# diver-j/melgan-multi

Measured on NVIDIA H100. Metric: generator_fwd_audio_frames_per_sec, higher is better.
Workload: dtype f32 in/out; products as 3 split-bf16 wgmma passes with fp32 accumulation (fp32-equivalent, ~1e-5)

## Files before the change

include/melgan_b200.h:

```cpp
#ifndef MELGAN_B200_H_
#define MELGAN_B200_H_

#include <stddef.h>
#include <stdint.h>

#ifdef __cplusplus
extern "C" {
#endif

#define MG_OK 0
#define MG_ERR_INVALID_ARGUMENT (-1)
#define MG_ERR_CUDA (-2)
#define MG_ERR_UNSUPPORTED_DEVICE (-3)
#define MG_ERR_WORKSPACE_TOO_SMALL (-4)
#define MG_ERR_OUT_OF_MEMORY (-5)

#define MG_GEN_NUM_LAYERS 30

int mg_abi_version(void);

const char *mg_last_error_string(void);

int mg_device_check(void);

// ... 8 lines not shown
#define MG_GEN_RAGGED_MAX_B 256
int mg_gen_forward_ragged(const void *packed, const float *mel, float *audio, int B, int T_max, const int *lengths,
                          void *workspace, size_t workspace_bytes, void *stream);

int mg_gen_forward_timed(const void *packed, const float *mel, float *audio, int B, int T,
                         void *workspace, size_t workspace_bytes, void *stream, float *kernel_ms);

int mg_gen_check_status(const void *workspace, int B, int T, void *stream);

int mg_gen_convt(const void *packed, int stage, const float *x, float *y, int B, int Lin, void *stream);

int mg_gen_resblock(const void *packed, int stage, const float *x, float *y, int B, int L, void *stream);
int mg_gen_upres(const void *packed, int stage, const float *x, float *y, int B, int Lin, void *stream);
int mg_gen_upres_post(const void *packed, const float *x, float *audio, int B, int Lin, void *stream);
const char *mg_gen_resblock_config(int code);

int mg_gen_resup(const void *packed, int stage, const float *x, float *y, int B, int L, void *stream);

int mg_gen_conv_pre(const void *packed, const float *mel, float *y, int B, int T, void *stream);
int mg_gen_resblock_post(const void *packed, const float *x, float *audio, int B, int L, void *stream);

int mg_gen_resblock_trace(const void *packed, int stage, const float *x, float *y, int B, int L, long long *trace_host);

int mg_gen_stage_output(const void *workspace, int which, float *out, int B, int T, void *stream);

size_t mg_msd_packed_bytes(void);
int mg_msd_pack(const float *const *v, const float *const *g, const float *const *bias, void *packed, void *stream);
int mg_msd_lengths(int L, int *lens);
int mg_msd_forward(const void *packed, const float *y, int Bt, int L, float *const *fmaps, void *status_word, void *stream);
int mg_msd_check_status(const void *status_word, void *stream);
// ... 65 lines not shown
```

melgan_multi_b200/csrc/mg_api.cu:

```cuda
#include <new>
#include <stdlib.h>
#include <string.h>

#include "mg_common.cuh"

namespace mg {


static int *status_ptr(void *workspace, int B, int T) {
    return reinterpret_cast<int *>(reinterpret_cast<float *>(workspace) + ws_offset(6, (size_t)B, (size_t)T));
}

static int run_generator(const float *packed, const float *mel, float *audio, const RunTable &batch, float *ws, cudaStream_t s,
                         cudaEvent_t *ev, const float *mel_host = nullptr, float *audio_host = nullptr) {
    int *st = status_ptr(ws, batch.items(), batch.stride);
    MG_CUDA_TRY(cudaMemsetAsync(st, 0, sizeof(int), s));
    return launch_generator_tc(packed, mel, audio, batch, ws, st, s, ev, mel_host, audio_host);
}

static int check_shape(const char *fn, int B, int T) {
    if (B < 1 || T < 1) return set_error(MG_ERR_INVALID_ARGUMENT, "%s: need B >= 1 and T >= 1 (got B=%d, T=%d)", fn, B, T);
    if ((long long)B * T > (1ll << 24)) return set_error(MG_ERR_INVALID_ARGUMENT, "%s: B*T = %lld too large", fn, (long long)B * T);
    return MG_OK;
}
// ... 264 lines not shown
int mg_gen_conv_pre(const void *packed, const float *mel, float *y, int B, int T, void *stream) {
    if (!packed || !mel || !y || B < 1 || T < 1) return set_error(MG_ERR_INVALID_ARGUMENT, "mg_gen_conv_pre: bad argument");
    return run_one_kernel("mg_gen_conv_pre", (cudaStream_t)stream, [&](int *st) {
        return launch_gen_pre_tc(mel, y, (const float *)packed, RunTable::uniform(B, T), st, (cudaStream_t)stream);
    });
}

int mg_gen_resblock_post(const void *packed, const float *x, float *audio, int B, int L, void *stream) {
    if (!packed || !x || !audio || B < 1 || L < 1) return set_error(MG_ERR_INVALID_ARGUMENT, "mg_gen_resblock_post: bad argument");
    return run_one_kernel("mg_gen_resblock_post", (cudaStream_t)stream, [&](int *st) {
        return launch_resblock_tc(x, audio, (const float *)packed, 4, RunTable::uniform(B, L), st, (cudaStream_t)stream);
    });
}

int mg_gen_resblock_trace(const void *packed, int stage, const float *x, float *y, int B, int L, long long *trace_host) {
    if (!packed || !x || !y || x == y || !trace_host || stage < 0 || stage > 3)
        return set_error(MG_ERR_INVALID_ARGUMENT, "mg_gen_resblock_trace: bad argument");
    int *st = nullptr;
    long long *tr = nullptr;
    MG_CUDA_TRY(cudaMalloc(&st, sizeof(int)));
    MG_CUDA_TRY(cudaMalloc(&tr, 128 * sizeof(long long)));
    cudaMemset(st, 0, sizeof(int));
    cudaMemset(tr, 0, 128 * sizeof(long long));
    int rc = launch_resblock_tc(x, y, (const float *)packed, stage, RunTable::uniform(B, L), st, 0, tr);
    if (rc == MG_OK && cudaDeviceSynchronize() != cudaSuccess) rc = set_error(MG_ERR_CUDA, "mg_gen_resblock_trace: kernel failed");
    if (rc == MG_OK) cudaMemcpy(trace_host, tr, 128 * sizeof(long long), cudaMemcpyDeviceToHost);
    cudaFree(st);
    cudaFree(tr);
    return rc;
}

// ... 18 lines not shown
        return set_error(MG_ERR_INVALID_ARGUMENT, "mg_gen_upres: bad argument");
    return run_one_kernel("mg_gen_upres", (cudaStream_t)stream, [&](int *st) {
        return launch_resblock_tc(x, y, (const float *)packed, 10 + stage, RunTable::uniform(B, 2 * Lin), st, (cudaStream_t)stream);
    });
}

int mg_gen_upres_post(const void *packed, const float *x, float *audio, int B, int Lin, void *stream) {
    if (!packed || !x || !audio || (const void *)x == (const void *)audio || B < 1 || Lin < 1)
        return set_error(MG_ERR_INVALID_ARGUMENT, "mg_gen_upres_post: bad argument");
    return run_one_kernel("mg_gen_upres_post", (cudaStream_t)stream, [&](int *st) {
        return launch_resblock_tc(x, audio, (const float *)packed, 14, RunTable::uniform(B, 2 * Lin), st, (cudaStream_t)stream);
    });
}

const char *mg_gen_resblock_config(int code) { return resblock_config_name(code, 0); }


size_t mg_msd_packed_bytes(void) { return msd_packed_bytes(); }

int mg_msd_pack(const float *const *v, const float *const *g, const float *const *bias, void *packed, void *stream) {
    if (!v || !g || !bias || !packed) return set_error(MG_ERR_INVALID_ARGUMENT, "mg_msd_pack: null argument");
    if ((uintptr_t)packed % 256) return set_error(MG_ERR_INVALID_ARGUMENT, "mg_msd_pack: packed must be 256-byte aligned");
    return launch_disc_pack(v, g, bias, packed, (cudaStream_t)stream);
}

int mg_msd_lengths(int L, int *lens) {
    if (L < 1 || !lens) return set_error(MG_ERR_INVALID_ARGUMENT, "mg_msd_lengths: bad argument");
    msd_lengths(L, lens);
    for (int i = 0; i < 21; ++i)
        if (lens[i] < 1) return set_error(MG_ERR_INVALID_ARGUMENT, "mg_msd_lengths: L = %d is too short for the discriminators", L);
// ... 192 lines not shown
```

melgan_multi_b200/csrc/mg_common.cuh:

```cuda
#pragma once
#include <cuda_runtime.h>
#include <stdarg.h>
#include <stdint.h>
#include <stdio.h>

#include "../../include/melgan_b200.h"
#include "mg_layout.h"

namespace mg {

constexpr int kNumSMs = 132;

char *error_buffer();
int set_error(int code, const char *fmt, ...);

#define MG_CUDA_TRY(expr)                                                                     \
    do {                                                                                      \
        cudaError_t err__ = (expr);                                                           \
        if (err__ != cudaSuccess)                                                             \
            return ::mg::set_error(MG_ERR_CUDA, "%s failed: %s (%s:%d)", #expr,               \
                                   cudaGetErrorString(err__), __FILE__, __LINE__);            \
    } while (0)

__device__ __forceinline__ float lrelu(float x) { return fmaxf(x, x * kSlope); }
// ... 150 lines not shown
                            float *const *dg, cudaStream_t s);
int launch_adam(float *const *p, const float *const *g, float *const *m, float *const *v, const long long *n, const int *first,
                int count, int total_ctas, float lr, float b1, float b2, float eps, float wd, long long step, cudaStream_t s);
long long loss_num_ctas(const long long *n, int count);
int launch_loss_forward(const float *const *a, const float *const *b, const long long *n, const int *mode, int count, float *out,
                        float *partial, cudaStream_t s);
int launch_loss_backward(const float *const *a, const float *const *b, const long long *n, const int *mode, int count,
                         const float *gout, float *const *ga, float *const *gb, cudaStream_t s);
struct MelTables;
size_t mel_tables_bytes();
int mel_tables_build(int sr, int n_mels, float fmin, float fmax, int norm, MelTables *t);
int mel_frames(int L);
int launch_mel(const void *tables, const float *audio, float *mel, int B, int L, cudaStream_t s);
int launch_msd_forward(const void *packed, const float *y, int Bt, int L, float *const *fmaps, int *status, cudaStream_t s);
int launch_convt_tc(const float *x, float *y, const float *packed, int stage, const RunTable &batch, int *status, cudaStream_t s);
int launch_resblock_tc(const float *x, float *y, const float *packed, int stage, const RunTable &batch, int *status, cudaStream_t s,
                       long long *trace = nullptr);

}
```

melgan_multi_b200/csrc/mg_res_tc.cu:

```cuda
#include <stdlib.h>
#include <string.h>

#include "mg_common.cuh"
#include "mg_tc.cuh"

namespace mg {
using namespace tc;

template <int C_, int NRB_, int RPW_, int NCP_, int NSTAGE_, bool POST_ = false, bool UPF_ = false, int UPT_ = 0, int CS_ = 1>
struct RbCfg {
    static constexpr int C = C_, NRB = NRB_, RPW = RPW_, NCP = NCP_, NSTAGE = NSTAGE_, UPT = UPT_, CS = CS_;
    static constexpr bool POST = POST_;
    static constexpr bool UPF = UPF_;
    static constexpr int P = 64 * NRB;
    static constexpr int NWG = NRB / RPW * NCP;
    static constexpr int NCONS = 128 * NWG;
    static constexpr int NT = NCONS + 32;
    static constexpr int NCW = C / NCP;
    static constexpr int SLACK = 16;
    static constexpr int HALO = 16 + (POST ? 3 : 0);
    static constexpr int HL = HALO + (UPT_ ? 1 : 0);
    static constexpr int ROWS = P + 2 * SLACK;
    static constexpr int XPITCH = ROWS * 16;
    static constexpr int KP = C / 8;
// ... 3 lines not shown
    static constexpr int HALF = CHUNK / 2;
    static constexpr int NCHUNK = tc_chunks_per_conv(C);
    static constexpr int KSL = C / KC;
    static constexpr int TNG = UPT == 8 ? 32 : C / 2, TN = (UPT ? UPT : 1) * TNG, TNCG = (C / 2) / TNG;
    static constexpr int TSLOT = UPT == 8 ? 16384 : 128 * UPT * TNG, TNSLOT = UPT ? TNCG * (C / 16) * (UPT == 8 ? 2 : 1) : 0;
    static_assert(UPT == 0 || ((UPT == 2 || UPT == 8) && TN == C && TSLOT <= CHUNK && !POST_ && !UPF_), "tail ConvT shape");
    static_assert(UPT != 8 || NCW == 128, "stride-8 tail: each column part stores four phases of a channel as one float4");
    static constexpr int UROWS = P / 2 + 2, UPITCH = UROWS * 16, NPB = NRB / 2, UKSL = 2 * C / KC, NUPCH = UPF ? 4 * UKSL : 0;
    static constexpr int SPITCH = P + 4;
    static_assert(!UPF || (NCP == 1 && NPB <= NWG && 2 * KP * UPITCH <= XBYTES && C * SPITCH * 4 <= 2 * XBYTES),
                  "fused ConvT must fit the X region");
    static_assert(!POST || (C == 32 && NCP == 1), "conv_post fusion is for the 32-channel stage");
    static constexpr int PVB = CS * P - HALO - HL, XCH = 9;
    static_assert(CS == 1 || ((CS == 2 || CS == 4) && !POST_ && !UPF_ && UPT_ == 0 && XCH <= SLACK && 2 * XCH <= P),
                  "clusters are for the plain ResBlock");
    static constexpr int SMEM_BYTES = 2 * XBYTES + NSTAGE * CHUNK + 2 * C * 4 + (2 * NSTAGE + (CS > 1 ? 2 : 0) + 1) * 8;
    static_assert(SMEM_BYTES + 1024 <= 227 * 1024, "shared memory budget");
    static_assert(XPITCH / 16 < 16384, "LBO field");
    static_assert(NRB % RPW == 0 && C % NCP == 0 && NCW % 32 == 0, "warpgroup split");
};

template <int RPW, int R>
__device__ __forceinline__ void acc_fence2(float (&a)[RPW][R]) {
#pragma unroll
    for (int r = 0; r < RPW; ++r) acc_fence<R>(a[r]);
}

template <class Cfg>
__global__ void __launch_bounds__(Cfg::NT, 1)
resblock_tc_kernel(const float *__restrict__ x, float *__restrict__ y, const float *__restrict__ packed, int stage,
                   const __grid_constant__ RunTable clusters, int *__restrict__ status, long long *__restrict__ trace) {
    constexpr int C = Cfg::C, P = Cfg::P, SLACK = Cfg::SLACK, HALO = Cfg::HALO, HL = Cfg::HL;
    constexpr int XPITCH = Cfg::XPITCH, XBYTES = Cfg::XBYTES, KC = Cfg::KC, CHUNK = Cfg::CHUNK, NSTAGE = Cfg::NSTAGE;
    constexpr int NCONS = Cfg::NCONS, NCP = Cfg::NCP, NCW = Cfg::NCW, RPW = Cfg::RPW, KSL = Cfg::KSL, NA = NCW / 2;
    constexpr int CS = Cfg::CS, XCH = Cfg::XCH;
    extern __shared__ __align__(1024) uint8_t smem[];
    uint8_t *Xh = smem, *Xl = smem + XBYTES, *ring = smem + 2 * XBYTES;
    float *pend = reinterpret_cast<float *>(ring + NSTAGE * CHUNK);
    float *b1s = pend + C;
    uint64_t *full = reinterpret_cast<uint64_t *>(b1s + C);
    uint64_t *empty = full + NSTAGE;
    uint64_t *hfull = empty + NSTAGE, *hfree = hfull + 1;
    int *item_len = reinterpret_cast<int *>(empty + NSTAGE + (CS > 1 ? 2 : 0));

    const int tid = threadIdx.x, warp = tid >> 5, lane = tid & 31;
    const int crank = blockIdx.x % CS;
    const RunPos cp = clusters.find(blockIdx.x / CS);
    const int clus = cp.unit, Ls = clusters.stride;
    auto item = [&]() { return *reinterpret_cast<volatile int *>(&item_len[0]); };
    auto len = [&]() { return *reinterpret_cast<volatile int *>(&item_len[1]); };
    const int oc = clus == 0 ? 0 : (CS * P - HALO) + (clus - 1) * Cfg::PVB - HL;
    const int o = oc + crank * P;
    const int p_lo = (clus == 0 || crank > 0) ? 0 : HL, p_hi = (crank < CS - 1 || oc + CS * P >= cp.len) ? P : P - HALO;
    const bool interior = (o >= 0 && o + P <= cp.len);
    const int l0 = 5 + 6 * stage;
// ... 6 lines not shown
            mbar_init(&full[s], 1);
            mbar_init(&empty[s], Cfg::NWG * CS);
        }
        if constexpr (CS > 1) {
            mbar_init(hfull, 1);
            mbar_init(hfree, (crank > 0) + (crank < CS - 1));
        }
        fence_mbar_init();
    }
    for (int i = Cfg::UPF ? 1 << 30 : tid; i < 2 * Cfg::KP * 2 * SLACK; i += Cfg::NT) {
        const int r = i % (2 * SLACK), kp = (i / (2 * SLACK)) % Cfg::KP, hl = i / (2 * SLACK * Cfg::KP);
        const int row = r < SLACK ? r : P + r;
        *reinterpret_cast<uint4 *>((hl ? Xl : Xh) + kp * XPITCH + row * 16) = make_uint4(0, 0, 0, 0);
    }
    for (int i = tid; i < C; i += Cfg::NT) pend[i] = 0.f;
    fence_proxy_async();
    __syncthreads();
    if constexpr (CS > 1) cluster_sync();
    const bool tr = trace && blockIdx.x == (gridDim.x > 1 ? 1u : 0u) && tid == 0;
#define MG_TR(slot) do { if (tr) trace[slot] = clock64(); } while (0)

    if (warp == NCONS / 32) {
        if (lane == 0) {
            int s = 0, ph = 0, j = 0;
            bool ok = true;
            auto put = [&](const uint8_t *src, uint32_t bytes) {
                if (!ok || !mbar_wait(&empty[s], ph ^ 1)) { ok = false; return; }
                mbar_arrive_expect_tx(&full[s], bytes);
                if constexpr (CS == 1) bulk_g2s(ring + s * CHUNK, src, bytes, &full[s]);
                else if (j % CS == crank) bulk_g2s_multicast(ring + s * CHUNK, src, bytes, &full[s], (1 << CS) - 1);
// ... 186 lines not shown
                    for (int k16 = 0; k16 < KC / 16; ++k16) {
                        const uint64_t bdesc = bbase + (uint64_t)(((pass == 2 ? Cfg::HALF : 0) + 2 * k16 * (C * 16)) >> 4);
                        const uint64_t adesc = desc_at(udesc_t, (pass == 1 ? xl_addr : xh_addr) + arow + 2 * k16 * UPITCH);
                        wgmma_bf16<NCW>(A[0], adesc, bdesc, !(k < 2 && ks == 0 && pass == 0 && k16 == 0));
                    }
                chunk_end();
            }
        };
        upf_tap(D, 0);
        upf_tap(R, 1);
        upf_tap(D, 2);
        upf_tap(R, 3);
        drain();
        sync_cons();
        float *stg = reinterpret_cast<float *>(Xh);
        const float *ubias = packed + bias_offset(1 + stage);
        if (mine) {
#pragma unroll
            for (int h = 0; h < 2; ++h) {
                const int m = wgi * 64 + frag_row(t, h);
#pragma unroll
                for (int j = 0; j < NA; ++j) {
                    const int col = frag_col(q, (j & ~3) | (j & 1));
                    if ((j & 2) == 2 * h) {
                        const float bj = __ldg(ubias + col);
                        *reinterpret_cast<float2 *>(stg + (size_t)col * SPITCH + 2 * m) = make_float2(R[0][j] + bj, D[0][j] + bj);
                    }
                }
            }
        }
        sync_cons();
#pragma unroll
        for (int r = 0; r < RPW; ++r)
#pragma unroll
            for (int j = 0; j < NA; ++j) {
                const int p = (rb0 + r) * 64 + frag_row(t, (j >> 1) & 1);
                R[r][j] = stg[(size_t)frag_col(q, (j & ~3) | (j & 1)) * SPITCH + p];
            }
        sync_cons();
        for (int i = tid; i < 2 * Cfg::KP * 2 * SLACK; i += NCONS) {
// ... 10 lines not shown
                const int p = (rb0 + r) * 64 + frag_row(t, h), tp = o + p;
                const bool inr = (tp >= 0 && tp < L);
                const float *xp = x + (size_t)b * C * Ls + (inr ? tp : 0);
#pragma unroll
                for (int k = 0; k < NCW / 8; ++k)
#pragma unroll
                    for (int e = 0; e < 2; ++e)
                        R[r][4 * k + 2 * h + e] = inr ? __ldg(xp + (size_t)(c0 + frag_col(q, 4 * k + e)) * Ls) : 0.f;
            }
    }
    hand_off(R, pend, false);
    MG_TR(1);

#pragma unroll 1
    for (int pr = 0; pr < 3; ++pr) {
        const float *bias1 = packed + bias_offset(l0 + pr);
        for (int c = tid; c < C; c += NCONS) b1s[c] = __ldg(bias1 + c);
        MG_TR(2 + 6 * pr);
        conv_mma(D, pr == 0 ? 1 : pr == 1 ? 3 : 9, true, 2 * pr);
        MG_TR(3 + 6 * pr);
        x_read();
        hand_off(D, b1s, false);
        MG_TR(4 + 6 * pr);
        const float *bias2 = packed + bias_offset(l0 + 3 + pr);
        for (int c = tid; c < C; c += NCONS) pend[c] += __ldg(bias2 + c);
        MG_TR(5 + 6 * pr);
        conv_mma(R, 1, false, 2 * pr + 1);
        MG_TR(6 + 6 * pr);
        x_read();
        if (pr < 2 || Cfg::UPT != 0) hand_off(R, pend, Cfg::UPT != 0 && pr == 2);
        MG_TR(7 + 6 * pr);
    }

    if constexpr (Cfg::POST) {
        pdl_trigger();
        float *Q = reinterpret_cast<float *>(Xh);
        float *wpost = reinterpret_cast<float *>(Xl);
        for (int i = tid; i < 32 * 8; i += NCONS)
            wpost[i] = (i & 7) < kPostK ? __ldg(packed + weight_offset(29) + (i >> 3) * kPostK + (i & 7)) : 0.f;
        sync_cons();
#pragma unroll
        for (int r = 0; r < RPW; ++r)
#pragma unroll
            for (int h = 0; h < 2; ++h) {
                const int p = (rb0 + r) * 64 + frag_row(t, h), tp = o + p;
                const bool inr = (tp >= 0 && tp < len());
                float qk[kPostK];
#pragma unroll
                for (int k = 0; k < kPostK; ++k) qk[k] = 0.f;
#pragma unroll
                for (int k = 0; k < NCW / 8; ++k)
#pragma unroll
                    for (int e = 0; e < 2; ++e) {
                        const int ci = frag_col(q, 4 * k + e);
                        const float a = inr ? lrelu(R[r][4 * k + 2 * h + e] + pend[ci]) : 0.f;
// ... 3 lines not shown
                        qk[3] = fmaf(w0.w, a, qk[3]); qk[4] = fmaf(w1.x, a, qk[4]); qk[5] = fmaf(w1.y, a, qk[5]);
                        qk[6] = fmaf(w1.z, a, qk[6]);
                    }
#pragma unroll
                for (int k = 0; k < kPostK; ++k) {
                    qk[k] += __shfl_xor_sync(0xffffffffu, qk[k], 1);
                    qk[k] += __shfl_xor_sync(0xffffffffu, qk[k], 2);
                }
                if (q == 0) {
#pragma unroll
                    for (int k = 0; k < kPostK; ++k) Q[k * P + p] = qk[k];
                }
            }
        sync_cons();
        const int b = item(), L = len();
        const float bpost = __ldg(packed + bias_offset(29));
#pragma unroll 1
        for (int p = tid; p < P; p += NCONS) {
            const int tp = o + p;
            if (p >= p_lo && p < p_hi && tp < L) {
                float acc = bpost;
#pragma unroll
                for (int k = 0; k < kPostK; ++k) {
                    const int pp = p + k - 3;
                    if (pp >= 0 && pp < P) acc += Q[k * P + pp];
                }
                y[(size_t)b * Ls + tp] = tanhf(acc);
            }
        }
        if (oc + P >= L)
            for (int p = L + tid; p < Ls; p += NCONS) y[(size_t)b * Ls + p] = 0.f;
    } else if constexpr (Cfg::UPT != 0) {
        constexpr int S = Cfg::UPT, TNG = Cfg::TNG, TN = Cfg::TN, PADT = S / 2, COT = C / 2;
        const int b = item(), L = len();
        const int Lout = S * Ls;
        const float *tbias = packed + bias_offset(1 + stage + 1);
        {
            const int pl = L - 1 - o;
            if (pl >= p_lo && pl < p_hi) {
                const float *wf = packed + weight_offset(1 + stage + 1);
                for (int i = tid; i < PADT * COT; i += NCONS) {
                    const int co = i / PADT, j = i - co * PADT;
                    const float *wp = wf + ((size_t)co * S + j) * 2 + 1;
                    float acc0 = 0.f, acc1 = 0.f, acc2 = 0.f, acc3 = 0.f;
#pragma unroll 1
                    for (int cc = 0; cc < C; cc += 32) {
                        float wv[32];
#pragma unroll
                        for (int k = 0; k < 32; ++k) wv[k] = __ldg(wp + (size_t)(cc + k) * COT * S * 2);
#pragma unroll
                        for (int k = 0; k < 32; k += 4) {
                            acc0 = fmaf(b1s[cc + k], wv[k], acc0);
                            acc1 = fmaf(b1s[cc + k + 1], wv[k + 1], acc1);
                            acc2 = fmaf(b1s[cc + k + 2], wv[k + 2], acc2);
                            acc3 = fmaf(b1s[cc + k + 3], wv[k + 3], acc3);
                        }
                    }
                    y[((size_t)b * COT + co) * Lout + (size_t)S * L - PADT + j] = (acc0 + acc1) + (acc2 + acc3) + __ldg(tbias + co);
                }
            }
        }
        const uint64_t tbdesc_t = desc_template(TN * 16, 128);
#pragma unroll 1
        for (int cg = 0; cg < Cfg::TNCG; ++cg) {
#pragma unroll 1
            for (int ch = 0; ch < C / 16; ++ch) {
#pragma unroll 1
                for (int ts = 0; ts < (S == 8 ? 2 : 1); ++ts) {
                    const uint64_t bbase = desc_at(tbdesc_t, chunk_begin() + c0 * 16);
#pragma unroll
                    for (int tp = 0; tp < (S == 8 ? 1 : 2); ++tp) {
                        const int tap = S == 8 ? ts : tp;
#pragma unroll
// ... 15 lines not shown
#pragma unroll
            for (int r = 0; r < RPW; ++r)
#pragma unroll
                for (int h = 0; h < 2; ++h) {
                    const int p = (rb0 + r) * 64 + frag_row(t, h), sg = o + p;
                    const bool own = (p >= p_lo && p < p_hi && sg < L);
                    const bool lo_ok = own && sg >= 1, hi_ok = own;
                    if constexpr (S == 8) {
                        const bool ok8 = c0 == 0 ? lo_ok : hi_ok;
                        float *yb = y + ((size_t)b * COT + cg * TNG) * Lout + (own ? 8 * sg - PADT + (c0 >> 5) : 0);
#pragma unroll
                        for (int c = 0; c < 4; ++c)
#pragma unroll
                            for (int e = 0; e < 2; ++e) {
                                const int co = 8 * c + 2 * q + e;
                                const float bj = __ldg(tbias + cg * TNG + co);
                                if (ok8)
                                    *reinterpret_cast<float4 *>(yb + (size_t)co * Lout) =
                                        make_float4(D[r][4 * c + 2 * h + e] + bj, D[r][4 * (4 + c) + 2 * h + e] + bj,
                                                    D[r][4 * (8 + c) + 2 * h + e] + bj, D[r][4 * (12 + c) + 2 * h + e] + bj);
                            }
                    } else {
                        float *yb = y + (size_t)b * COT * Lout + (own ? 2 * sg - PADT : 0);
#pragma unroll
                        for (int k = 0; k < NCW / 8; ++k)
#pragma unroll
                            for (int e = 0; e < 2; ++e) {
                                const int col = c0 + frag_col(q, 4 * k + e), phi = col / TNG, co = col % TNG;
                                if (phi == 0 ? lo_ok : hi_ok) yb[(size_t)co * Lout + phi] = D[r][4 * k + 2 * h + e] + __ldg(tbias + co);
                            }
                    }
                }
        }
    } else {
        pdl_trigger();
        const int b = item(), L = len();
#pragma unroll
        for (int r = 0; r < RPW; ++r)
#pragma unroll
            for (int h = 0; h < 2; ++h) {
                const int p = (rb0 + r) * 64 + frag_row(t, h), tp = o + p;
                if (p >= p_lo && p < p_hi && tp < L) {
                    float *yp = y + (size_t)b * C * Ls + tp;
#pragma unroll
// ... 106 lines not shown
```

melgan_multi_b200/csrc/mg_up_tc.cu:

```cuda
#include "mg_common.cuh"
#include "mg_tc.cuh"

namespace mg {
using namespace tc;

template <int STAGE_>
struct UpCfg {
    static constexpr int STAGE = STAGE_;
    static constexpr int CIN = stage_cin(STAGE), COUT = stage_cout(STAGE), S = stage_stride(STAGE), PAD = stage_pad(STAGE);
    static constexpr int NG = up_ng(STAGE);
    static constexpr int NCG = COUT / NG;
    static constexpr int N = S * NG;
    static constexpr int NMW = (N > 128) ? 1 : 2;
    static constexpr int KCA = (S == 8) ? 64 : 32;
    static constexpr int ROWS = 64 * NMW;
    static constexpr int AROWS = ROWS + 8;
    static constexpr int APITCH = AROWS * 16;
    static constexpr int ASLOT = 2 * (KCA / 8) * APITCH;
    static constexpr int BSLOT = up_slot_bytes(STAGE);
    static constexpr int NSA = (CIN == KCA) ? 1 : 2, NSB = (S == 8) ? 4 : (CIN >= 128 ? 2 : 3);
    static constexpr int NCHUNK = CIN / 16;
    static constexpr int NCONV = 128;
    static constexpr int NT = NCONV + 128 * NMW + 32;
    static constexpr int SMEM_BYTES = NSA * ASLOT + NSB * BSLOT + (2 * NSA + 2 * NSB) * 8;
    static_assert(N <= 256 && N % 16 == 0, "wgmma N");
    static_assert(SMEM_BYTES + 1024 <= 227 * 1024, "shared memory budget");
    static_assert(CIN % KCA == 0, "A slot");
};

template <class Cfg, class Row>
__device__ __forceinline__ void convt_store(const float *acc, float *__restrict__ y, const float *__restrict__ bias, int mw, int t,
                                            int cg, int Lout, Row row) {
    constexpr int S = Cfg::S, NG = Cfg::NG, N = Cfg::N, COUT = Cfg::COUT, PAD = Cfg::PAD;
    const int q = t & 3;
#pragma unroll
    for (int h = 0; h < 2; ++h) {
        int m = 64 * mw + frag_row(t, h);
        asm volatile("" : "+r"(m) : : "memory");
        const RunPos p = row(m);
        const int s = p.unit;
        const bool row_ok = p.item >= 0;
        const bool lo_ok = row_ok && s >= 1, hi_ok = row_ok && s <= p.len - 1;
        float *yb = y + ((size_t)(row_ok ? p.item : 0) * COUT + cg * NG) * Lout + (S * s - PAD);
        if constexpr (S == 8) {
#pragma unroll
            for (int c = 0; c < 4; ++c)
#pragma unroll
                for (int e = 0; e < 2; ++e) {
                    const int co = 8 * c + 2 * q + e;
                    const float bj = __ldg(bias + co);
                    float *yp = yb + (size_t)co * Lout;
                    if (lo_ok)
                        *reinterpret_cast<float4 *>(yp) =
                            make_float4(acc[4 * (0 + c) + 2 * h + e] + bj, acc[4 * (4 + c) + 2 * h + e] + bj,
                                        acc[4 * (8 + c) + 2 * h + e] + bj, acc[4 * (12 + c) + 2 * h + e] + bj);
                    if (hi_ok)
                        *reinterpret_cast<float4 *>(yp + 4) =
                            make_float4(acc[4 * (16 + c) + 2 * h + e] + bj, acc[4 * (20 + c) + 2 * h + e] + bj,
                                        acc[4 * (24 + c) + 2 * h + e] + bj, acc[4 * (28 + c) + 2 * h + e] + bj);
                }
        } else {
#pragma unroll
            for (int k = 0; k < N / 8; ++k)
#pragma unroll
                for (int e = 0; e < 2; ++e) {
                    const int col = frag_col(q, 4 * k + e), phi = col / NG, co = col % NG;
                    const float o = acc[4 * k + 2 * h + e] + __ldg(bias + co);
                    if (phi == 0 ? lo_ok : hi_ok) yb[(size_t)co * Lout + phi] = o;
                }
        }
    }
}

template <class Cfg>
__global__ void __launch_bounds__(Cfg::NT, 1)
convt_tc_kernel(const float *__restrict__ x, float *__restrict__ y, const float *__restrict__ packed,
                const __grid_constant__ RunTable rows, int *__restrict__ status) {
    constexpr int CIN = Cfg::CIN, N = Cfg::N, NG = Cfg::NG;
    constexpr int ROWS = Cfg::ROWS, APITCH = Cfg::APITCH, ASLOT = Cfg::ASLOT, BSLOT = Cfg::BSLOT, KCA = Cfg::KCA;
    constexpr int NSA = Cfg::NSA, NSB = Cfg::NSB, NCHUNK = Cfg::NCHUNK, NCONV = Cfg::NCONV, NMW = Cfg::NMW;
    extern __shared__ __align__(1024) uint8_t smem[];
    uint8_t *aring = smem, *bring = smem + NSA * ASLOT;
    uint64_t *fullA = reinterpret_cast<uint64_t *>(bring + NSB * BSLOT);
    uint64_t *emptyA = fullA + NSA, *fullB = emptyA + NSA, *emptyB = fullB + NSB;

// ... 105 lines not shown
    rows.set_units([](int Lin) { return Lin + 1; });
    return rows;
}

template <class Cfg>
static int launch_convt(const float *x, float *y, const float *packed, const RunTable &batch, int *status, cudaStream_t s) {
    static bool configured = false;
    if (!configured) {
        MG_CUDA_TRY(cudaFuncSetAttribute(convt_tc_kernel<Cfg>, cudaFuncAttributeMaxDynamicSharedMemorySize, Cfg::SMEM_BYTES));
        configured = true;
    }
    const RunTable rows = convt_rows(batch);
    dim3 grid((unsigned)((rows.first[rows.n] + Cfg::ROWS - 1) / Cfg::ROWS), Cfg::NCG);
    MG_CUDA_TRY(launch_ex(convt_tc_kernel<Cfg>, grid, dim3(Cfg::NT), Cfg::SMEM_BYTES, s, true, 1, x, y, packed, rows, status));
    return MG_OK;
}

template <class Cfg>
__global__ void __launch_bounds__(Cfg::NCONV + 128 + 32, 1)
convt_resident_tc_kernel(const float *__restrict__ x, float *__restrict__ y, const float *__restrict__ packed,
                         const __grid_constant__ RunTable rows, int *__restrict__ status) {
    constexpr int CIN = Cfg::CIN, NG = Cfg::NG, N = Cfg::N, NCG = Cfg::NCG;
    constexpr int ROWS = 64, APITCH = Cfg::APITCH, BSLOT = Cfg::BSLOT, NCHUNK = Cfg::NCHUNK;
    constexpr int KPT = CIN / 8;
    constexpr int AHALF = KPT * APITCH;
    constexpr int NSB = 4, NCONV = Cfg::NCONV;
    static_assert(Cfg::S == 8 && N == 256 && Cfg::NMW == 1 && 2 * AHALF + NSB * BSLOT + 256 + ROWS * 12 <= 227 * 1024,
                  "resident ConvT shape");
    extern __shared__ __align__(1024) uint8_t smem[];
    uint8_t *abuf = smem, *bring = smem + 2 * AHALF;
// ... 98 lines not shown
    static bool configured = false;
    if (!configured) {
        MG_CUDA_TRY(cudaFuncSetAttribute(convt_resident_tc_kernel<Cfg>, cudaFuncAttributeMaxDynamicSharedMemorySize, smem));
        configured = true;
    }
    const RunTable rows = convt_rows(batch);
    MG_CUDA_TRY(launch_ex(convt_resident_tc_kernel<Cfg>, dim3((unsigned)((rows.first[rows.n] + 63) / 64)), dim3(Cfg::NCONV + 128 + 32),
                          smem, s, true, 1, x, y, packed, rows, status));
    return MG_OK;
}

int launch_convt_tc(const float *x, float *y, const float *packed, int stage, const RunTable &batch, int *status, cudaStream_t s) {
    switch (stage) {
        case 0: return launch_convt<UpCfg<0>>(x, y, packed, batch, status, s);
        case 1: return launch_convt_resident<UpCfg<1>>(x, y, packed, batch, status, s);
        case 2: return launch_convt<UpCfg<2>>(x, y, packed, batch, status, s);
        case 3: return launch_convt<UpCfg<3>>(x, y, packed, batch, status, s);
    }
    return set_error(MG_ERR_INVALID_ARGUMENT, "launch_convt_tc: stage %d", stage);
}

}
```

melgan_multi_b200/engine.py:

```python
import ctypes
import os

import numpy as np

_HERE = os.path.dirname(os.path.abspath(__file__))
LIB_PATH = os.path.join(_HERE, "lib", "libmelgan_b200.so")
NUM_LAYERS = 30

_f32p = ctypes.POINTER(ctypes.c_float)
_lib = None


class EngineError(RuntimeError):
    pass


def lib():
    global _lib
    if _lib is None:
        if not os.path.exists(LIB_PATH):
            raise EngineError(
                "libmelgan_b200.so is not built (%s). Run `python -m melgan_multi_b200.build` "
                "(needs nvcc); there is no CPU/PyTorch fallback for the hot path." % LIB_PATH)
        L = ctypes.CDLL(LIB_PATH)
# ... 16 lines not shown
        L.mg_gen_check_status.restype = ctypes.c_int
        L.mg_gen_check_status.argtypes = [ctypes.c_void_p, ctypes.c_int, ctypes.c_int, ctypes.c_void_p]
        L.mg_gen_convt.restype = ctypes.c_int
        L.mg_gen_convt.argtypes = [ctypes.c_void_p, ctypes.c_int, ctypes.c_void_p, ctypes.c_void_p, ctypes.c_int,
                                   ctypes.c_int, ctypes.c_void_p]
        L.mg_gen_resblock.restype = ctypes.c_int
        L.mg_gen_resblock.argtypes = [ctypes.c_void_p, ctypes.c_int, ctypes.c_void_p, ctypes.c_void_p, ctypes.c_int,
                                      ctypes.c_int, ctypes.c_void_p]
        L.mg_gen_upres.restype = ctypes.c_int
        L.mg_gen_upres.argtypes = [ctypes.c_void_p, ctypes.c_int, ctypes.c_void_p, ctypes.c_void_p, ctypes.c_int,
                                   ctypes.c_int, ctypes.c_void_p]
        L.mg_gen_upres_post.restype = ctypes.c_int
        L.mg_gen_upres_post.argtypes = [ctypes.c_void_p] * 3 + [ctypes.c_int, ctypes.c_int, ctypes.c_void_p]
        L.mg_gen_resblock_config.restype = ctypes.c_char_p
        L.mg_gen_resblock_config.argtypes = [ctypes.c_int]
        L.mg_gen_conv_pre.restype = ctypes.c_int
        L.mg_gen_conv_pre.argtypes = [ctypes.c_void_p, ctypes.c_void_p, ctypes.c_void_p, ctypes.c_int, ctypes.c_int, ctypes.c_void_p]
        L.mg_gen_resblock_post.restype = ctypes.c_int
        L.mg_gen_resblock_post.argtypes = [ctypes.c_void_p, ctypes.c_void_p, ctypes.c_void_p, ctypes.c_int, ctypes.c_int, ctypes.c_void_p]
        L.mg_disc_packed_bytes.restype = ctypes.c_size_t
        L.mg_disc_pack.restype = ctypes.c_int
        L.mg_disc_pack.argtypes = [ctypes.c_void_p] * 5
        L.mg_disc_forward.restype = ctypes.c_int
        L.mg_disc_forward.argtypes = [ctypes.c_void_p, ctypes.c_void_p, ctypes.c_int, ctypes.c_int, ctypes.c_void_p,
                                      ctypes.c_void_p, ctypes.c_void_p]
        L.mg_gen_resup.restype = ctypes.c_int
        L.mg_gen_resup.argtypes = [ctypes.c_void_p, ctypes.c_int, ctypes.c_void_p, ctypes.c_void_p, ctypes.c_int, ctypes.c_int,
                                   ctypes.c_void_p]
        L.mg_gen_set_pipeline.restype = ctypes.c_int
        L.mg_gen_set_pipeline.argtypes = [ctypes.c_int]
# ... 647 lines not shown
```

Baseline: 256.2 million.

## Add persistent streaming ConvT kernel for stride-2 stages and cache resblock constants in smem

Replaces the stride-2 transposed-conv launches for stages 2 and 3 with a persistent kernel. It keeps all weights resident in shared memory, streams input tiles through a bulk-copy staging ring, converts them to split-bf16 in producer warps, and stores paired outputs with warp shuffles. Separately, the resblock kernel preloads every bias and the conv_post weights into shared memory once, instead of issuing __ldg reads inside each phase. The aim is to cut weight reloads per tile, launch and tail overhead, and scattered global constant reads, at the cost of more shared memory and more complex segment and ragged-row handling.

```diff
diff --git a/include/melgan_b200.h b/include/melgan_b200.h
--- a/include/melgan_b200.h
+++ b/include/melgan_b200.h
@@ -46,6 +46,7 @@
 int mg_gen_upres(const void *packed, int stage, const float *x, float *y, int B, int Lin, void *stream);
 int mg_gen_upres_post(const void *packed, const float *x, float *audio, int B, int Lin, void *stream);
 const char *mg_gen_resblock_config(int code);
+const char *mg_gen_convt_config(int stage);
 
 int mg_gen_resup(const void *packed, int stage, const float *x, float *y, int B, int L, void *stream);
 
diff --git a/melgan_multi_b200/csrc/mg_api.cu b/melgan_multi_b200/csrc/mg_api.cu
--- a/melgan_multi_b200/csrc/mg_api.cu
+++ b/melgan_multi_b200/csrc/mg_api.cu
@@ -302,7 +302,7 @@
 }
 
 int mg_gen_resblock_trace(const void *packed, int stage, const float *x, float *y, int B, int L, long long *trace_host) {
-    if (!packed || !x || !y || x == y || !trace_host || stage < 0 || stage > 3)
+    if (!packed || !x || !y || x == y || !trace_host || !*resblock_config_name(stage, 0) || B < 1 || L < 1)
         return set_error(MG_ERR_INVALID_ARGUMENT, "mg_gen_resblock_trace: bad argument");
     int *st = nullptr;
     long long *tr = nullptr;
@@ -351,6 +351,7 @@
 }
 
 const char *mg_gen_resblock_config(int code) { return resblock_config_name(code, 0); }
+const char *mg_gen_convt_config(int stage) { return convt_config_name(stage); }
 
 
 size_t mg_msd_packed_bytes(void) { return msd_packed_bytes(); }
diff --git a/melgan_multi_b200/csrc/mg_common.cuh b/melgan_multi_b200/csrc/mg_common.cuh
--- a/melgan_multi_b200/csrc/mg_common.cuh
+++ b/melgan_multi_b200/csrc/mg_common.cuh
@@ -188,6 +188,7 @@
 int launch_mel(const void *tables, const float *audio, float *mel, int B, int L, cudaStream_t s);
 int launch_msd_forward(const void *packed, const float *y, int Bt, int L, float *const *fmaps, int *status, cudaStream_t s);
 int launch_convt_tc(const float *x, float *y, const float *packed, int stage, const RunTable &batch, int *status, cudaStream_t s);
+const char *convt_config_name(int stage);
 int launch_resblock_tc(const float *x, float *y, const float *packed, int stage, const RunTable &batch, int *status, cudaStream_t s,
                        long long *trace = nullptr);
 
diff --git a/melgan_multi_b200/csrc/mg_res_tc.cu b/melgan_multi_b200/csrc/mg_res_tc.cu
--- a/melgan_multi_b200/csrc/mg_res_tc.cu
+++ b/melgan_multi_b200/csrc/mg_res_tc.cu
@@ -41,7 +41,10 @@
     static constexpr int PVB = CS * P - HALO - HL, XCH = 9;
     static_assert(CS == 1 || ((CS == 2 || CS == 4) && !POST_ && !UPF_ && UPT_ == 0 && XCH <= SLACK && 2 * XCH <= P),
                   "clusters are for the plain ResBlock");
-    static constexpr int SMEM_BYTES = 2 * XBYTES + NSTAGE * CHUNK + 2 * C * 4 + (2 * NSTAGE + (CS > 1 ? 2 : 0) + 1) * 8;
+    static constexpr int CB_UPF = 6 * C, CB_UPT = CB_UPF + (UPF_ ? C : 0), CB_POST = CB_UPT + (UPT_ ? C / 2 : 0);
+    static constexpr int NCONST = CB_POST + (POST_ ? 32 * 8 + 4 : 0);
+    static_assert(CB_POST % 4 == 0 && NCONST % 2 == 0, "conv_post weights are read as float4, the mbarriers follow");
+    static constexpr int SMEM_BYTES = 2 * XBYTES + NSTAGE * CHUNK + (2 * C + NCONST) * 4 + (2 * NSTAGE + (CS > 1 ? 2 : 0) + 1) * 8;
     static_assert(SMEM_BYTES + 1024 <= 227 * 1024, "shared memory budget");
     static_assert(XPITCH / 16 < 16384, "LBO field");
     static_assert(NRB % RPW == 0 && C % NCP == 0 && NCW % 32 == 0, "warpgroup split");
@@ -65,7 +68,8 @@
     uint8_t *Xh = smem, *Xl = smem + XBYTES, *ring = smem + 2 * XBYTES;
     float *pend = reinterpret_cast<float *>(ring + NSTAGE * CHUNK);
     float *b1s = pend + C;
-    uint64_t *full = reinterpret_cast<uint64_t *>(b1s + C);
+    float *cst = b1s + C;
+    uint64_t *full = reinterpret_cast<uint64_t *>(cst + Cfg::NCONST);
     uint64_t *empty = full + NSTAGE;
     uint64_t *hfull = empty + NSTAGE, *hfree = hfull + 1;
     int *item_len = reinterpret_cast<int *>(empty + NSTAGE + (CS > 1 ? 2 : 0));
@@ -102,6 +106,19 @@
         *reinterpret_cast<uint4 *>((hl ? Xl : Xh) + kp * XPITCH + row * 16) = make_uint4(0, 0, 0, 0);
     }
     for (int i = tid; i < C; i += Cfg::NT) pend[i] = 0.f;
+    for (int i = tid; i < Cfg::NCONST; i += Cfg::NT) {
+        float v = 0.f;
+        if (i < Cfg::CB_UPF) v = __ldg(packed + bias_offset(l0) + i);
+        else if (i < Cfg::CB_UPT) v = __ldg(packed + bias_offset(1 + stage) + (i - Cfg::CB_UPF));
+        else if (i < Cfg::CB_POST) v = __ldg(packed + bias_offset(1 + stage + 1) + (i - Cfg::CB_UPT));
+        else if (i < Cfg::CB_POST + 32 * 8) {
+            const int j = i - Cfg::CB_POST;
+            if ((j & 7) < kPostK) v = __ldg(packed + weight_offset(29) + (j >> 3) * kPostK + (j & 7));
+        } else if (i == Cfg::CB_POST + 32 * 8) {
+            v = __ldg(packed + bias_offset(29));
+        }
+        cst[i] = v;
+    }
     fence_proxy_async();
     __syncthreads();
     if constexpr (CS > 1) cluster_sync();
@@ -318,7 +335,7 @@
         drain();
         sync_cons();
         float *stg = reinterpret_cast<float *>(Xh);
-        const float *ubias = packed + bias_offset(1 + stage);
+        const float *ubias = cst + Cfg::CB_UPF;
         if (mine) {
 #pragma unroll
             for (int h = 0; h < 2; ++h) {
@@ -327,7 +344,7 @@
                 for (int j = 0; j < NA; ++j) {
                     const int col = frag_col(q, (j & ~3) | (j & 1));
                     if ((j & 2) == 2 * h) {
-                        const float bj = __ldg(ubias + col);
+                        const float bj = ubias[col];
                         *reinterpret_cast<float2 *>(stg + (size_t)col * SPITCH + 2 * m) = make_float2(R[0][j] + bj, D[0][j] + bj);
                     }
                 }
@@ -368,16 +385,13 @@
 
 #pragma unroll 1
     for (int pr = 0; pr < 3; ++pr) {
-        const float *bias1 = packed + bias_offset(l0 + pr);
-        for (int c = tid; c < C; c += NCONS) b1s[c] = __ldg(bias1 + c);
         MG_TR(2 + 6 * pr);
         conv_mma(D, pr == 0 ? 1 : pr == 1 ? 3 : 9, true, 2 * pr);
         MG_TR(3 + 6 * pr);
         x_read();
-        hand_off(D, b1s, false);
+        hand_off(D, cst + pr * C, false);
         MG_TR(4 + 6 * pr);
-        const float *bias2 = packed + bias_offset(l0 + 3 + pr);
-        for (int c = tid; c < C; c += NCONS) pend[c] += __ldg(bias2 + c);
+        for (int c = tid; c < C; c += NCONS) pend[c] += cst[(3 + pr) * C + c];
         MG_TR(5 + 6 * pr);
         conv_mma(R, 1, false, 2 * pr + 1);
         MG_TR(6 + 6 * pr);
@@ -389,10 +403,7 @@
     if constexpr (Cfg::POST) {
         pdl_trigger();
         float *Q = reinterpret_cast<float *>(Xh);
-        float *wpost = reinterpret_cast<float *>(Xl);
-        for (int i = tid; i < 32 * 8; i += NCONS)
-            wpost[i] = (i & 7) < kPostK ? __ldg(packed + weight_offset(29) + (i >> 3) * kPostK + (i & 7)) : 0.f;
-        sync_cons();
+        const float *wpost = cst + Cfg::CB_POST;
 #pragma unroll
         for (int r = 0; r < RPW; ++r)
 #pragma unroll
@@ -426,7 +437,7 @@
             }
         sync_cons();
         const int b = item(), L = len();
-        const float bpost = __ldg(packed + bias_offset(29));
+        const float bpost = cst[Cfg::CB_POST + 32 * 8];
 #pragma unroll 1
         for (int p = tid; p < P; p += NCONS) {
             const int tp = o + p;
@@ -446,7 +457,7 @@
         constexpr int S = Cfg::UPT, TNG = Cfg::TNG, TN = Cfg::TN, PADT = S / 2, COT = C / 2;
         const int b = item(), L = len();
         const int Lout = S * Ls;
-        const float *tbias = packed + bias_offset(1 + stage + 1);
+        const float *tbias = cst + Cfg::CB_UPT;
         {
             const int pl = L - 1 - o;
             if (pl >= p_lo && pl < p_hi) {
@@ -468,7 +479,7 @@
                             acc3 = fmaf(b1s[cc + k + 3], wv[k + 3], acc3);
                         }
                     }
-                    y[((size_t)b * COT + co) * Lout + (size_t)S * L - PADT + j] = (acc0 + acc1) + (acc2 + acc3) + __ldg(tbias + co);
+                    y[((size_t)b * COT + co) * Lout + (size_t)S * L - PADT + j] = (acc0 + acc1) + (acc2 + acc3) + tbias[co];
                 }
             }
         }
@@ -514,7 +525,7 @@
 #pragma unroll
                             for (int e = 0; e < 2; ++e) {
                                 const int co = 8 * c + 2 * q + e;
-                                const float bj = __ldg(tbias + cg * TNG + co);
+                                const float bj = tbias[cg * TNG + co];
                                 if (ok8)
                                     *reinterpret_cast<float4 *>(yb + (size_t)co * Lout) =
                                         make_float4(D[r][4 * c + 2 * h + e] + bj, D[r][4 * (4 + c) + 2 * h + e] + bj,
@@ -527,7 +538,7 @@
 #pragma unroll
                             for (int e = 0; e < 2; ++e) {
                                 const int col = c0 + frag_col(q, 4 * k + e), phi = col / TNG, co = col % TNG;
-                                if (phi == 0 ? lo_ok : hi_ok) yb[(size_t)co * Lout + phi] = D[r][4 * k + 2 * h + e] + __ldg(tbias + co);
+                                if (phi == 0 ? lo_ok : hi_ok) yb[(size_t)co * Lout + phi] = D[r][4 * k + 2 * h + e] + tbias[co];
                             }
                     }
                 }
diff --git a/melgan_multi_b200/csrc/mg_up_tc.cu b/melgan_multi_b200/csrc/mg_up_tc.cu
--- a/melgan_multi_b200/csrc/mg_up_tc.cu
+++ b/melgan_multi_b200/csrc/mg_up_tc.cu
@@ -18,7 +18,7 @@
     static constexpr int APITCH = AROWS * 16;
     static constexpr int ASLOT = 2 * (KCA / 8) * APITCH;
     static constexpr int BSLOT = up_slot_bytes(STAGE);
-    static constexpr int NSA = (CIN == KCA) ? 1 : 2, NSB = (S == 8) ? 4 : (CIN >= 128 ? 2 : 3);
+    static constexpr int NSA = (CIN == KCA) ? 1 : 2, NSB = 4;
     static constexpr int NCHUNK = CIN / 16;
     static constexpr int NCONV = 128;
     static constexpr int NT = NCONV + 128 * NMW + 32;
@@ -31,7 +31,8 @@
 template <class Cfg, class Row>
 __device__ __forceinline__ void convt_store(const float *acc, float *__restrict__ y, const float *__restrict__ bias, int mw, int t,
                                             int cg, int Lout, Row row) {
-    constexpr int S = Cfg::S, NG = Cfg::NG, N = Cfg::N, COUT = Cfg::COUT, PAD = Cfg::PAD;
+    constexpr int S = Cfg::S, NG = Cfg::NG, COUT = Cfg::COUT, PAD = Cfg::PAD;
+    static_assert(S == 8, "the stride-2 stages store through convt_stream_store");
     const int q = t & 3;
 #pragma unroll
     for (int h = 0; h < 2; ++h) {
@@ -42,33 +43,22 @@
         const bool row_ok = p.item >= 0;
         const bool lo_ok = row_ok && s >= 1, hi_ok = row_ok && s <= p.len - 1;
         float *yb = y + ((size_t)(row_ok ? p.item : 0) * COUT + cg * NG) * Lout + (S * s - PAD);
-        if constexpr (S == 8) {
-#pragma unroll
-            for (int c = 0; c < 4; ++c)
-#pragma unroll
-                for (int e = 0; e < 2; ++e) {
-                    const int co = 8 * c + 2 * q + e;
-                    const float bj = __ldg(bias + co);
-                    float *yp = yb + (size_t)co * Lout;
-                    if (lo_ok)
-                        *reinterpret_cast<float4 *>(yp) =
-                            make_float4(acc[4 * (0 + c) + 2 * h + e] + bj, acc[4 * (4 + c) + 2 * h + e] + bj,
-                                        acc[4 * (8 + c) + 2 * h + e] + bj, acc[4 * (12 + c) + 2 * h + e] + bj);
-                    if (hi_ok)
-                        *reinterpret_cast<float4 *>(yp + 4) =
-                            make_float4(acc[4 * (16 + c) + 2 * h + e] + bj, acc[4 * (20 + c) + 2 * h + e] + bj,
-                                        acc[4 * (24 + c) + 2 * h + e] + bj, acc[4 * (28 + c) + 2 * h + e] + bj);
-                }
-        } else {
-#pragma unroll
-            for (int k = 0; k < N / 8; ++k)
-#pragma unroll
-                for (int e = 0; e < 2; ++e) {
-                    const int col = frag_col(q, 4 * k + e), phi = col / NG, co = col % NG;
-                    const float o = acc[4 * k + 2 * h + e] + __ldg(bias + co);
-                    if (phi == 0 ? lo_ok : hi_ok) yb[(size_t)co * Lout + phi] = o;
-                }
-        }
+#pragma unroll
+        for (int c = 0; c < 4; ++c)
+#pragma unroll
+            for (int e = 0; e < 2; ++e) {
+                const int co = 8 * c + 2 * q + e;
+                const float bj = __ldg(bias + co);
+                float *yp = yb + (size_t)co * Lout;
+                if (lo_ok)
+                    *reinterpret_cast<float4 *>(yp) =
+                        make_float4(acc[4 * (0 + c) + 2 * h + e] + bj, acc[4 * (4 + c) + 2 * h + e] + bj,
+                                    acc[4 * (8 + c) + 2 * h + e] + bj, acc[4 * (12 + c) + 2 * h + e] + bj);
+                if (hi_ok)
+                    *reinterpret_cast<float4 *>(yp + 4) =
+                        make_float4(acc[4 * (16 + c) + 2 * h + e] + bj, acc[4 * (20 + c) + 2 * h + e] + bj,
+                                    acc[4 * (24 + c) + 2 * h + e] + bj, acc[4 * (28 + c) + 2 * h + e] + bj);
+            }
     }
 }
 
@@ -204,6 +194,272 @@
     dim3 grid((unsigned)((rows.first[rows.n] + Cfg::ROWS - 1) / Cfg::ROWS), Cfg::NCG);
     MG_CUDA_TRY(launch_ex(convt_tc_kernel<Cfg>, grid, dim3(Cfg::NT), Cfg::SMEM_BYTES, s, true, 1, x, y, packed, rows, status));
     return MG_OK;
+}
+
+template <class Cfg>
+struct StreamCfg {
+    static_assert(Cfg::S == 2 && Cfg::NCG == 1 && Cfg::NMW == 2, "streaming ConvT: stride 2, one channel group");
+    static constexpr int MAXSEG = 3;
+    static constexpr int AR = Cfg::ROWS + 1;
+    static constexpr int XPITCH = (AR + 6 * MAXSEG + 3) & ~3;
+    static constexpr int XSLOT = Cfg::KCA * XPITCH * 4;
+    static constexpr int BRES = Cfg::NCHUNK * Cfg::BSLOT;
+    static constexpr int NSA = 2;
+    static constexpr int FIXED = BRES + NSA * Cfg::ASLOT + 256;
+    static constexpr int NSX = (227 * 1024 - 1024 - FIXED) / XSLOT < 4 ? (227 * 1024 - 1024 - FIXED) / XSLOT : 4;
+    static constexpr int NT = Cfg::NCONV + 128 * Cfg::NMW + 32;
+    static constexpr int SMEM_BYTES = BRES + NSA * Cfg::ASLOT + NSX * XSLOT + (1 + 2 * NSA + 2 * NSX) * 8;
+    static_assert(NSX >= 2 && SMEM_BYTES + 1024 <= 227 * 1024, "shared memory budget");
+    static_assert(XPITCH % 4 == 0 && Cfg::KCA == 32, "staging slot: 16-byte channel rows, one channel per producer lane");
+};
+
+struct XSeg {
+    int i0, n, item, u0, dst;
+};
+template <class SC>
+__device__ __forceinline__ void tile_segments(const RunTable &rows, int r0, XSeg (&seg)[SC::MAXSEG], int &covered) {
+    int i = r0 == 0 ? 1 : 0, dst = 0;
+#pragma unroll
+    for (int k = 0; k < SC::MAXSEG; ++k) {
+        RunPos p = rows.find(r0 - 1 + i);
+        if (i < SC::AR && p.item >= 0 && p.unit == p.len) p = rows.find(r0 - 1 + ++i);
+        const int n = (i < SC::AR && p.item >= 0) ? min(p.len - p.unit, SC::AR - i) : 0;
+        seg[k] = {i, n, p.item, p.unit, dst};
+        dst += (n + 6) & ~3;
+        i += n;
+    }
+    covered = i;
+}
+
+template <class Cfg>
+__device__ __forceinline__ void convt_stream_store(const float *acc, const float (&bj)[Cfg::NG / 8][2], float *__restrict__ y, int mw,
+                                                   int t, int r0, const RunTable &rows) {
+    constexpr int KB = Cfg::NG / 8, COUT = Cfg::COUT;
+    const int lane = t & 31, q = t & 3, g = lane >> 2;
+    const int Lout = 2 * rows.stride;
+#pragma unroll
+    for (int h = 0; h < 2; ++h) {
+        int m = 64 * mw + frag_row(t, h);
+        asm volatile("" : "+r"(m) : : "memory");
+        const RunPos p = rows.find(r0 + m);
+        const int s = p.unit;
+        const bool pair_ok = p.item >= 0 && s < p.len, lo_ok = p.item >= 0 && s >= 1;
+        float *yb = y + (size_t)(p.item >= 0 ? p.item : 0) * COUT * Lout + 2 * s;
+#pragma unroll
+        for (int k = 0; k < KB; ++k)
+#pragma unroll
+            for (int e = 0; e < 2; ++e) {
+                const int co = 8 * k + 2 * q + e;
+                const float p0 = acc[4 * k + 2 * h + e] + bj[k][e];
+                const float p1 = acc[4 * (KB + k) + 2 * h + e] + bj[k][e];
+                const float nx = h == 0 ? __shfl_sync(0xffffffffu, g == 0 ? acc[4 * k + 2 + e] + bj[k][e] : p0, (lane + 4) & 31)
+                                        : __shfl_down_sync(0xffffffffu, p0, 4);
+                float *yp = yb + (size_t)co * Lout;
+                if (h == 1 && g == 7) {
+                    if (pair_ok) yp[0] = p1;
+                } else if (pair_ok) {
+                    *reinterpret_cast<float2 *>(yp) = make_float2(p1, nx);
+                }
+                if (h == 0 && g == 0 && lo_ok) yp[-1] = p0;
+            }
+    }
+}
+
+template <class Cfg>
+__global__ void __launch_bounds__(StreamCfg<Cfg>::NT, 1)
+convt_stream_tc_kernel(const float *__restrict__ x, float *__restrict__ y, const float *__restrict__ packed,
+                       const __grid_constant__ RunTable rows, int ntiles, int *__restrict__ status) {
+    using SC = StreamCfg<Cfg>;
+    constexpr int CIN = Cfg::CIN, N = Cfg::N, NG = Cfg::NG, KCA = Cfg::KCA, NCONV = Cfg::NCONV, NMW = Cfg::NMW;
+    constexpr int ROWS = Cfg::ROWS, APITCH = Cfg::APITCH, ASLOT = Cfg::ASLOT, BSLOT = Cfg::BSLOT, NCHUNK = Cfg::NCHUNK;
+    constexpr int AR = SC::AR, XPITCH = SC::XPITCH, XSLOT = SC::XSLOT, NSA = SC::NSA, NSX = SC::NSX, MAXSEG = SC::MAXSEG;
+    extern __shared__ __align__(1024) uint8_t smem[];
+    uint8_t *bres = smem, *aring = smem + SC::BRES, *xring = aring + NSA * ASLOT;
+    uint64_t *fullW = reinterpret_cast<uint64_t *>(xring + NSX * XSLOT);
+    uint64_t *fullA = fullW + 1, *emptyA = fullA + NSA, *fullX = emptyA + NSA, *emptyX = fullX + NSX;
+
+    const int tid = threadIdx.x, warp = tid >> 5, lane = tid & 31;
+    const int Lin = rows.stride;
+
+    if (tid == 0) {
+        mbar_init(fullW, 1);
+        for (int s = 0; s < NSA; ++s) { mbar_init(&fullA[s], NCONV); mbar_init(&emptyA[s], NMW); }
+        for (int s = 0; s < NSX; ++s) { mbar_init(&fullX[s], 1); mbar_init(&emptyX[s], NCONV); }
+        fence_mbar_init();
+    }
+    __syncthreads();
+
+    if (warp == (NCONV + 128 * NMW) / 32) {
+        if (lane == 0) {
+            const uint8_t *src = reinterpret_cast<const uint8_t *>(packed) + tc_region_start() + tc_up_offset(Cfg::STAGE);
+            mbar_arrive_expect_tx(fullW, SC::BRES);
+            for (int i = 0; i < NCHUNK; ++i) bulk_g2s(bres + i * BSLOT, src + (size_t)i * BSLOT, BSLOT, fullW);
+        }
+        pdl_wait();
+        int sx = 0, phx = 0;
+        bool ok = true;
+#pragma unroll 1
+        for (int tile = blockIdx.x; tile < ntiles && ok; tile += gridDim.x) {
+            const int r0 = tile * ROWS;
+            XSeg seg[MAXSEG];
+            int covered;
+            tile_segments<SC>(rows, r0, seg, covered);
+#pragma unroll 1
+            for (int ca = 0; ca < CIN / KCA; ++ca) {
+                ok = __shfl_sync(0xffffffffu, lane == 0 ? mbar_wait(&emptyX[sx], phx ^ 1) : false, 0);
+                if (!ok) break;
+                float *slot = reinterpret_cast<float *>(xring + sx * XSLOT) + lane * XPITCH;
+                size_t g0[MAXSEG];
+                uint32_t bytes = 0;
+#pragma unroll
+                for (int k = 0; k < MAXSEG; ++k) {
+                    g0[k] = ((size_t)seg[k].item * CIN + ca * KCA + lane) * Lin + seg[k].u0;
+                    if (seg[k].n > 0) bytes += (uint32_t)((((g0[k] + seg[k].n + 3) & ~(size_t)3) - (g0[k] & ~(size_t)3)) * 4);
+                }
+                const uint32_t total = __reduce_add_sync(0xffffffffu, bytes);
+                if (lane == 0) mbar_arrive_expect_tx(&fullX[sx], total);
+                __syncwarp();
+#pragma unroll
+                for (int k = 0; k < MAXSEG; ++k)
+                    if (seg[k].n > 0) {
+                        const size_t a = g0[k] & ~(size_t)3, e = (g0[k] + seg[k].n + 3) & ~(size_t)3;
+                        bulk_g2s(slot + seg[k].dst, x + a, (uint32_t)((e - a) * 4), &fullX[sx]);
+                    }
+                if (++sx == NSX) { sx = 0; phx ^= 1; }
+            }
+        }
+        if (!ok && lane == 0) atomicExch(status, 12);
+    } else if (warp >= NCONV / 32) {
+        const int mw = warp / 4 - NCONV / 128, t = tid & 127;
+        const uint64_t adesc_t = desc_template(APITCH, 128), bdesc_t = desc_template(N * 16, 128);
+        const uint32_t aring_addr = smem_u32(aring) + mw * 64 * 16, bres_addr = smem_u32(bres);
+        float bj[NG / 8][2];
+#pragma unroll
+        for (int k = 0; k < NG / 8; ++k)
+#pragma unroll
+            for (int e = 0; e < 2; ++e) bj[k][e] = __ldg(packed + bias_offset(1 + Cfg::STAGE) + 8 * k + 2 * (t & 3) + e);
+        float acc[N / 2];
+        int sa = 0, pha = 0;
+        bool ok = mbar_wait(fullW, 0);
+#pragma unroll 1
+        for (int tile = blockIdx.x; tile < ntiles; tile += gridDim.x) {
+            int psa = -1;
+#pragma unroll 1
+            for (int ca = 0; ca < CIN / KCA; ++ca) {
+                ok &= mbar_wait(&fullA[sa], pha);
+                const uint64_t abase = desc_at(adesc_t, aring_addr + sa * ASLOT);
+#pragma unroll 1
+                for (int j = 0; j < KCA / 16; ++j) {
+                    const uint64_t bbase = desc_at(bdesc_t, bres_addr + (ca * (KCA / 16) + j) * BSLOT);
+                    wgmma_fence();
+#pragma unroll
+                    for (int tap = 0; tap < 2; ++tap)
+#pragma unroll
+                        for (int pass = 0; pass < 3; ++pass) {
+                            const int ahalf = (pass == 1), bhalf = (pass == 2);
+                            const uint64_t bdesc = bbase + (uint64_t)((((tap * 2 + bhalf) * 2) * N * 16) >> 4);
+                            const uint64_t adesc = abase + (uint64_t)((ahalf * (KCA / 8) * APITCH + (1 - tap) * 16) >> 4) +
+                                                   (uint64_t)(2 * j * (APITCH >> 4));
+                            wgmma_bf16<N>(acc, adesc, bdesc, (ca | j | tap | pass) != 0);
+                        }
+                    wgmma_commit();
+                    wgmma_wait<1>();
+                    if (t == 0 && psa >= 0) mbar_arrive(&emptyA[psa]);
+                    psa = (j == KCA / 16 - 1) ? sa : -1;
+                }
+                if (++sa == NSA) { sa = 0; pha ^= 1; }
+            }
+            wgmma_wait<0>();
+            acc_fence<N / 2>(acc);
+            if (t == 0) mbar_arrive(&emptyA[psa]);
+            if (tile + (int)gridDim.x >= ntiles) pdl_trigger();
+            pdl_wait();
+            convt_stream_store<Cfg>(acc, bj, y, mw, t, tile * ROWS, rows);
+        }
+        if (!ok && t == 0) atomicExch(status, 13);
+    } else {
+        pdl_wait();
+        int sx = 0, phx = 0, sa = 0, pha = 0;
+        bool ok = true;
+#pragma unroll 1
+        for (int tile = blockIdx.x; tile < ntiles; tile += gridDim.x) {
+            const int r0 = tile * ROWS;
+            XSeg seg[MAXSEG];
+            int covered;
+            tile_segments<SC>(rows, r0, seg, covered);
+#pragma unroll 1
+            for (int ca = 0; ca < CIN / KCA; ++ca) {
+                if (ok && !(mbar_wait(&fullX[sx], phx) && mbar_wait(&emptyA[sa], pha ^ 1))) {
+                    ok = false;
+                    atomicExch(status, 14);
+                }
+                const float *xs = reinterpret_cast<const float *>(xring + sx * XSLOT);
+                uint8_t *slot = aring + sa * ASLOT;
+#pragma unroll 1
+                for (int u = tid; u < AR * (KCA / 8); u += NCONV) {
+                    const int i = u % AR, kp = u / AR;
+                    int off = -1;
+                    uint32_t gb = 0;
+#pragma unroll
+                    for (int k = 0; k < MAXSEG; ++k)
+                        if (i >= seg[k].i0 && i < seg[k].i0 + seg[k].n) {
+                            off = seg[k].dst + i - seg[k].i0;
+                            gb = ((uint32_t)seg[k].item * CIN + ca * KCA + 8 * kp) * (uint32_t)Lin + seg[k].u0;
+                        }
+                    float f[8];
+                    if (off >= 0) {
+#pragma unroll
+                        for (int e = 0; e < 8; ++e) f[e] = xs[(8 * kp + e) * XPITCH + off + ((gb + e * Lin) & 3)];
+                    } else {
+                        const RunPos p = i >= covered ? rows.find(r0 - 1 + i) : RunPos{-1, 0, 0};
+                        const bool inr = p.item >= 0 && p.unit < p.len;
+                        const float *xp = x + ((size_t)(inr ? p.item : 0) * CIN + ca * KCA + 8 * kp) * Lin + (inr ? p.unit : 0);
+#pragma unroll
+                        for (int e = 0; e < 8; ++e) f[e] = inr ? __ldg(xp + (size_t)e * Lin) : 0.f;
+                    }
+                    uint32_t h[4], l[4];
+#pragma unroll
+                    for (int e = 0; e < 4; ++e) split2_bf16(lrelu(f[2 * e]), lrelu(f[2 * e + 1]), h[e], l[e]);
+                    *reinterpret_cast<uint4 *>(slot + kp * APITCH + i * 16) = make_uint4(h[0], h[1], h[2], h[3]);
+                    *reinterpret_cast<uint4 *>(slot + (KCA / 8 + kp) * APITCH + i * 16) = make_uint4(l[0], l[1], l[2], l[3]);
+                }
+                fence_proxy_async();
+                mbar_arrive(&fullA[sa]);
+                mbar_arrive(&emptyX[sx]);
+                if (++sa == NSA) { sa = 0; pha ^= 1; }
+                if (++sx == NSX) { sx = 0; phx ^= 1; }
+            }
+        }
+    }
+}
+
+template <class Cfg>
+static int launch_convt_stream(const float *x, float *y, const float *packed, const RunTable &batch, int *status, cudaStream_t s) {
+    using SC = StreamCfg<Cfg>;
+    static bool configured = false;
+    if (!configured) {
+        MG_CUDA_TRY(cudaFuncSetAttribute(convt_stream_tc_kernel<Cfg>, cudaFuncAttributeMaxDynamicSharedMemorySize, SC::SMEM_BYTES));
+        configured = true;
+    }
+    if (reinterpret_cast<uintptr_t>(x) % 16 != 0)
+        return set_error(MG_ERR_INVALID_ARGUMENT, "launch_convt_tc: stage %d input not 16-byte aligned", Cfg::STAGE);
+    int dev = 0, sms = 0;
+    MG_CUDA_TRY(cudaGetDevice(&dev));
+    MG_CUDA_TRY(cudaDeviceGetAttribute(&sms, cudaDevAttrMultiProcessorCount, dev));
+    const RunTable rows = convt_rows(batch);
+    const int ntiles = (rows.first[rows.n] + Cfg::ROWS - 1) / Cfg::ROWS;
+    const unsigned grid = (unsigned)(ntiles < sms ? ntiles : sms);
+    MG_CUDA_TRY(launch_ex(convt_stream_tc_kernel<Cfg>, dim3(grid), dim3(SC::NT), SC::SMEM_BYTES, s, true, 1, x, y, packed, rows, ntiles,
+                          status));
+    return MG_OK;
+}
+
+template <class Cfg>
+static const char *stream_cfg_name() {
+    static char buf[80];
+    snprintf(buf, sizeof(buf), "convt_stream_tc_kernel<StreamCfg<%d,%d,%d,%d>>", Cfg::STAGE, Cfg::ROWS, StreamCfg<Cfg>::MAXSEG,
+             StreamCfg<Cfg>::NSX);
+    return buf;
 }
 
 template <class Cfg>
@@ -332,10 +588,18 @@
     switch (stage) {
         case 0: return launch_convt<UpCfg<0>>(x, y, packed, batch, status, s);
         case 1: return launch_convt_resident<UpCfg<1>>(x, y, packed, batch, status, s);
-        case 2: return launch_convt<UpCfg<2>>(x, y, packed, batch, status, s);
-        case 3: return launch_convt<UpCfg<3>>(x, y, packed, batch, status, s);
+        case 2: return launch_convt_stream<UpCfg<2>>(x, y, packed, batch, status, s);
+        case 3: return launch_convt_stream<UpCfg<3>>(x, y, packed, batch, status, s);
     }
     return set_error(MG_ERR_INVALID_ARGUMENT, "launch_convt_tc: stage %d", stage);
 }
 
-}
+const char *convt_config_name(int stage) {
+    switch (stage) {
+        case 2: return stream_cfg_name<UpCfg<2>>();
+        case 3: return stream_cfg_name<UpCfg<3>>();
+    }
+    return "";
+}
+
+}
diff --git a/melgan_multi_b200/engine.py b/melgan_multi_b200/engine.py
--- a/melgan_multi_b200/engine.py
+++ b/melgan_multi_b200/engine.py
@@ -54,6 +54,8 @@
         L.mg_gen_upres_post.argtypes = [ctypes.c_void_p] * 3 + [ctypes.c_int, ctypes.c_int, ctypes.c_void_p]
         L.mg_gen_resblock_config.restype = ctypes.c_char_p
         L.mg_gen_resblock_config.argtypes = [ctypes.c_int]
+        L.mg_gen_convt_config.restype = ctypes.c_char_p
+        L.mg_gen_convt_config.argtypes = [ctypes.c_int]
         L.mg_gen_conv_pre.restype = ctypes.c_int
         L.mg_gen_conv_pre.argtypes = [ctypes.c_void_p, ctypes.c_void_p, ctypes.c_void_p, ctypes.c_int, ctypes.c_int, ctypes.c_void_p]
         L.mg_gen_resblock_post.restype = ctypes.c_int
```

Measured after the change: 277.7 million, median of 6. 1.08x the previous value.
